# Lalwaniamisha789/Implementation-of-Neural-LDPC-Decoders-with-Degree-Specific-Weight-Sharing-and-RCQ-Quantization

Measured on AMD Instinct MI355X. Metric: decoded codewords/sec at fixed iters; achieved HBM GB/s vs peak, higher is better.
Workload: dtype f32; 1 GPU; (1998,1512) IRA code, BasicMinSumDecoder factor=0.7, fp32, 10 iterations, batch 65536/GPU, SNR 2.0 dB, fixed-iteration flooding decode; graph=ira_1998_1512, n=1998, m=486, edges=6587, batch_per_gpu=65536, global_batch=65536, parallelism=dp1, collective=none

## Files before the change

implementation-of-neural-ldpc-decoders-with-degree-specific-weight-sharing-and-rcq-quantization_amd/_native.py:

```python

from __future__ import annotations

import ctypes as C
import os
import subprocess
import threading
from typing import Optional

import numpy as np

_HERE = os.path.dirname(os.path.abspath(__file__))
LIB_NAME = "libldpc_hip.so"
LIB_PATH = os.environ.get("LDPC_HIP_LIB") or os.path.join(_HERE, LIB_NAME)
CSRC = os.path.join(_HERE, "csrc")
HEADER = os.path.join(os.path.dirname(_HERE), "include", "ldpc_hip.h")
DEBUG_HEADER = os.path.join(os.path.dirname(_HERE), "include", "ldpc_hip_debug.h")

LDPC_F32, LDPC_F64 = 0, 1
C2V_NMS, C2V_RCQ, C2V_OMS = 0, 1, 2
MODE_AUTO, MODE_STREAM, MODE_RESIDENT, MODE_SWEEPS, MODE_GATHER, MODE_PAIR = 0, 1, 2, 3, 4, 5
SCHED_FLOODING, SCHED_LAYERED_REF, SCHED_LAYERED = 0, 1, 2

HIPCC_FLAGS = ["--offload-arch=gfx950", "-O3", "-std=c++17", "-fPIC", "-shared",
               "-ffp-contract=off",
# ... 29 lines not shown
        fn = lib.ldpc_source_hash
        fn.restype = C.c_char_p
        fn.argtypes = []
        return fn().decode() or None
    except (OSError, AttributeError):
        return None


def is_stale(target: Optional[str] = None, defines=()) -> bool:
    target = target or os.path.join(_HERE, LIB_NAME)
    return not os.path.exists(target) or built_hash(target) != source_hash(defines)


def build_native(force: bool = False, verbose: bool = False, defines=(), out: Optional[str] = None) -> str:
    srcs = _source_files()
    target = out or os.path.join(_HERE, LIB_NAME)
    want = source_hash(defines)
    if not force and os.path.exists(target) and built_hash(target) == want:
        return target
    hipcc = os.environ.get("HIPCC") or ("/opt/rocm/bin/hipcc" if os.path.exists("/opt/rocm/bin/hipcc") else "hipcc")
    tmp = target + ".tmp%d" % os.getpid()
    cmd = [hipcc] + HIPCC_FLAGS + [f"-D{d}" for d in defines] + [f"-DLDPC_SRC_HASH={want}", "-o", tmp, srcs[0]]
    res = subprocess.run(cmd, capture_output=True, text=True)
    if verbose or res.returncode != 0:
        print(" ".join(cmd))
        print(res.stdout + res.stderr)
    if res.returncode != 0:
        try:
            os.unlink(tmp)
        except OSError:
            pass
        raise NativeEngineError("hipcc failed:\n" + res.stderr[-4000:])
    os.replace(tmp, target)
    return target


class DecoderDesc(C.Structure):
    _fields_ = [("dtype", C.c_int32), ("c2v_form", C.c_int32), ("iters", C.c_int32),
                ("n_beta_slots", C.c_int32), ("beta", C.c_void_p), ("beta_slot", C.c_void_p),
                ("n_alpha_slots", C.c_int32), ("alpha", C.c_void_p), ("alpha_slot", C.c_void_p),
                ("n_levels", C.c_int32), ("n_quantizers", C.c_int32), ("thresholds", C.c_void_p),
                ("q_of_iter", C.c_void_p),
                ("n_oms_alpha_slots", C.c_int32), ("oms_alpha", C.c_void_p), ("oms_alpha_slot", C.c_void_p),
                ("schedule", C.c_int32)]


PRODUCT_EXPORTS = ("ldpc_graph_create", "ldpc_graph_destroy", "ldpc_graph_info", "ldpc_decoder_create",
                   "ldpc_decoder_set_mode", "ldpc_decoder_info",
                   "ldpc_decoder_set_weights", "ldpc_decoder_destroy", "ldpc_decoder_workspace_bytes",
                   "ldpc_decode", "ldpc_decode_capped", "ldpc_last_error", "ldpc_abi_version", "ldpc_source_hash",
                   "ldpc_train_saved_bytes", "ldpc_train_workspace_bytes", "ldpc_decode_saving", "ldpc_backward",
                   "ldpc_train_joint_workspace_bytes", "ldpc_train_joint")
DEBUG_EXPORTS = ("ldpc_debug_sweep", "ldpc_debug_workspace_layout", "ldpc_debug_resident_c2v", "ldpc_debug_key4",
                 "ldpc_debug_compact_layout", "ldpc_debug_compact_checks")
EXPORTS = PRODUCT_EXPORTS + DEBUG_EXPORTS

_lib = None
_lock = threading.Lock()


def load():
    global _lib
    if _lib is not None:
        return _lib
    with _lock:
        if _lib is not None:
            return _lib
        if not os.path.exists(LIB_PATH):
            raise NativeEngineError(
                f"{LIB_NAME} is not built: run `python -c 'import __graft_entry__ as g; g.build()'` "
                f"(hipcc --offload-arch=gfx950) -- there is no CPU fallback for the decode path")
        if "LDPC_HIP_LIB" not in os.environ and is_stale(LIB_PATH):
            raise NativeEngineError(
                f"{LIB_PATH} was not built from the sources in csrc/ (content hash {built_hash(LIB_PATH)} != "
                f"{source_hash()}): run `python -c 'import __graft_entry__ as g; g.build()'` -- a stale engine is never loaded")
        try:
            lib = C.CDLL(LIB_PATH)
        except OSError as e:
            raise NativeEngineError(f"cannot load {LIB_PATH}: {e}") from e
        vp, i32, i64 = C.c_void_p, C.c_int32, C.c_int64
        lib.ldpc_graph_create.restype = C.c_int
        lib.ldpc_graph_create.argtypes = [C.POINTER(vp), i32, i32, i32, vp, vp]
        lib.ldpc_graph_destroy.restype = None
        lib.ldpc_graph_destroy.argtypes = [vp]
        lib.ldpc_graph_info.restype = C.c_int
        lib.ldpc_graph_info.argtypes = [vp, vp]
        lib.ldpc_decoder_create.restype = C.c_int
        lib.ldpc_decoder_create.argtypes = [C.POINTER(vp), vp, C.POINTER(DecoderDesc)]
        lib.ldpc_decoder_set_mode.restype = C.c_int
        lib.ldpc_decoder_set_mode.argtypes = [vp, i32]
        lib.ldpc_decoder_info.restype = C.c_int
        lib.ldpc_decoder_info.argtypes = [vp, vp]
        lib.ldpc_decoder_set_weights.restype = C.c_int
        lib.ldpc_decoder_set_weights.argtypes = [vp, vp, vp, vp, vp]
        lib.ldpc_decoder_destroy.restype = None
        lib.ldpc_decoder_destroy.argtypes = [vp]
        lib.ldpc_decoder_workspace_bytes.restype = C.c_size_t
        lib.ldpc_decoder_workspace_bytes.argtypes = [vp, i64]
        lib.ldpc_decode.restype = C.c_int
        lib.ldpc_decode.argtypes = [vp, vp, i64, i32, vp, vp, vp, vp, vp, vp, C.c_size_t, vp]
        lib.ldpc_decode_capped.restype = C.c_int
        lib.ldpc_decode_capped.argtypes = [vp, vp, i64, i32, i32, vp, vp, vp, vp, vp, vp, C.c_size_t, vp]
        lib.ldpc_debug_sweep.restype = C.c_int
        lib.ldpc_debug_sweep.argtypes = [vp, i64, i32, i32, vp, C.c_size_t, vp]
        lib.ldpc_debug_workspace_layout.restype = C.c_int
        lib.ldpc_debug_workspace_layout.argtypes = [vp, i64, i32, vp]
        lib.ldpc_debug_key4.restype = C.c_int
        lib.ldpc_debug_key4.argtypes = [vp, i64, C.c_float, vp, vp, vp, vp]
        lib.ldpc_debug_resident_c2v.restype = C.c_int
        lib.ldpc_debug_resident_c2v.argtypes = [vp, vp, i64, i32, i32, vp, vp, vp, vp]
        lib.ldpc_debug_compact_layout.restype = C.c_int
        lib.ldpc_debug_compact_layout.argtypes = [vp, i32, i32, i32, vp, vp, vp, vp, vp]
        lib.ldpc_debug_compact_checks.restype = C.c_int
        lib.ldpc_debug_compact_checks.argtypes = [vp, i32, i32, i32, vp, vp, vp]
        lib.ldpc_train_saved_bytes.restype = C.c_size_t
        lib.ldpc_train_saved_bytes.argtypes = [vp, i64]
        lib.ldpc_train_workspace_bytes.restype = C.c_size_t
        lib.ldpc_train_workspace_bytes.argtypes = [vp, i64]
        lib.ldpc_decode_saving.restype = C.c_int
        lib.ldpc_decode_saving.argtypes = [vp, vp, i64, i32, vp, vp, vp, vp, vp, C.c_size_t, vp, C.c_size_t, vp]
        lib.ldpc_backward.restype = C.c_int
        lib.ldpc_backward.argtypes = [vp, vp, C.c_size_t, vp, i64, vp, vp, vp, vp, vp, vp, vp, C.c_size_t, vp]
        lib.ldpc_train_joint_workspace_bytes.restype = C.c_size_t
        lib.ldpc_train_joint_workspace_bytes.argtypes = [vp, i64]
        lib.ldpc_train_joint.restype = C.c_int
        lib.ldpc_train_joint.argtypes = [vp, vp, vp, i64, vp, vp, vp, vp, vp, vp, vp, vp, vp, C.c_size_t, vp]
        lib.ldpc_last_error.restype = C.c_char_p
        lib.ldpc_last_error.argtypes = []
        lib.ldpc_abi_version.restype = C.c_int
        lib.ldpc_abi_version.argtypes = []
        lib.ldpc_source_hash.restype = C.c_char_p
        lib.ldpc_source_hash.argtypes = []
        if lib.ldpc_abi_version() != 1:
            raise NativeEngineError("libldpc_hip.so ABI version mismatch")
        _lib = lib
    return _lib


def check(rc: int, what: str):
    if rc != 0:
        msg = load().ldpc_last_error().decode(errors="replace")
        if rc == -3:
            raise NotImplementedError(f"{what}: {msg}")
        if rc == -1:
            raise ValueError(f"{what}: {msg}")
        raise NativeEngineError(f"{what} failed (rc={rc}): {msg}")


def ptr(a: Optional[np.ndarray]):
    return None if a is None else a.ctypes.data_as(C.c_void_p)
```

implementation-of-neural-ldpc-decoders-with-degree-specific-weight-sharing-and-rcq-quantization_amd/csrc/ldpc_hip.hip:

```cpp
#include "ldpc_kernels.hip"
#include "ldpc_resident.hip"
#include "ldpc_train.hip"
#include "ldpc_layered.hip"

#include <algorithm>
#include <climits>
#include <mutex>
#include <set>
#include <cmath>
#include <cstdarg>
#include <cstdio>
#include <cstdlib>
#include <cstring>
#include <exception>
#include <new>
#include <vector>

#include "../../include/ldpc_hip.h"
#include "../../include/ldpc_hip_debug.h"

using namespace ldpc;

namespace {

// ... 5 lines not shown
    va_start(ap, fmt);
    vsnprintf(g_err, sizeof(g_err), fmt, ap);
    va_end(ap);
    return code;
}

#define HIP_TRY(expr)                                                                         \
    do {                                                                                      \
        hipError_t e_ = (expr);                                                               \
        if (e_ != hipSuccess) return fail(LDPC_ERR_HIP, "%s -> %s", #expr, hipGetErrorString(e_)); \
    } while (0)

constexpr size_t kAlign = 256;
size_t align_up(size_t x) { return (x + kAlign - 1) / kAlign * kAlign; }

template <typename X>
int upload(X **dst, const X *src, size_t count)
{
    *dst = nullptr;
    if (count == 0) count = 1;
    HIP_TRY(hipMalloc((void **)dst, count * sizeof(X)));
    if (src) HIP_TRY(hipMemcpy(*dst, src, count * sizeof(X), hipMemcpyHostToDevice));
    return LDPC_OK;
}

struct DeviceGuard {
    int prev = -1;
    bool switched = false;
    explicit DeviceGuard(int dev)
    {
        if (hipGetDevice(&prev) == hipSuccess && prev != dev) switched = hipSetDevice(dev) == hipSuccess;
    }
    ~DeviceGuard()
    {
        if (switched) (void)hipSetDevice(prev);
    }
};

}

struct ldpc_graph {
    int device = 0;
    int n = 0, m = 0, E = 0, max_dc = 0, max_dv = 0;
    int *check_ptr = nullptr, *var_idx = nullptr, *var_ptr = nullptr, *csc_edge = nullptr;
    int *wide_checks = nullptr;
    int n_wide = 0;
    std::vector<int> h_check_ptr, h_var_idx, h_var_ptr, h_csc, h_check_of_edge;
    GraphDev dev() const { return GraphDev{n, m, E, check_ptr, var_idx, var_ptr, csc_edge}; }
};

constexpr int kCptWaves = kResCptThreads / 64;
constexpr int kCptCells = kCptWaves * kResRegVars;
constexpr int kCptMaxDv = 8;
inline int cpt_body_cost(int dv) { return dv * (dv - 1) + 2 * dv + 4; }

struct CptLayout {
    std::vector<int> var_at;
    unsigned cell[kCptWaves] = {};
    int worst = 0, total = 0;
    int mixed = 0;
};

struct ldpc_decoder {
    const ldpc_graph *g = nullptr;
    int dtype = LDPC_F32, form = LDPC_C2V_NMS, T = 0;
    int n_beta = 0, n_alpha = 0, n_levels = 0, n_quant = 0, n_oms_alpha = 0;
    void *beta = nullptr, *alpha = nullptr, *oms_alpha = nullptr;
    int *beta_slot = nullptr, *alpha_slot = nullptr, *oms_alpha_slot = nullptr;
    float *thresholds = nullptr;
    float *lut = nullptr;
    std::vector<int> q_of_iter;
    int *q_of_iter_dev = nullptr;
    size_t elem() const { return dtype == LDPC_F64 ? 8 : 4; }
    int schedule = 0;
    int mode = 0;
    bool res_ok = false;
    int res_G = 0, res_NT = 0;
    bool unit_alpha = false, rcq_zero0 = false;
    bool beta_per_check = false;
    size_t res_lds = 0;
    ResidentPlan res{};
    bool resc_ok = false;
    size_t resc_lds = 0;
    ResidentPlan resc{};
    CptLayout resc_layout;
    std::vector<void *> res_bufs;
    int *beta_inv_ptr = nullptr, *beta_inv_items = nullptr;
    int *alpha_inv_ptr = nullptr, *alpha_inv_items = nullptr;
    int *oms_inv_ptr = nullptr, *oms_inv_items = nullptr;
    bool gat_ok = false;
    bool pair_ok = false;
    bool key_float4 = false;
    int4 *gat_meta = nullptr;
    int *gat_nbr = nullptr;
    bool lay_ok = false;
    LayeredPlan lay{};
    uint32_t *lay_off = nullptr;
    size_t lay_lds = 0;
    int *lay_slot = nullptr;
    float *lay_beta = nullptr;
    bool beta_unit = false;
};

namespace {

bool use_resident(const ldpc_decoder *d) { return d->res_ok && (d->mode == LDPC_MODE_AUTO || d->mode == LDPC_MODE_RESIDENT); }
bool use_layered_lds(const ldpc_decoder *d) { return d->lay_ok && (d->mode == LDPC_MODE_AUTO || d->mode == LDPC_MODE_RESIDENT); }
bool use_pair(const ldpc_decoder *d) { return d->pair_ok && d->mode != LDPC_MODE_SWEEPS && d->mode != LDPC_MODE_GATHER; }
bool use_gather(const ldpc_decoder *d) { return d->gat_ok && !use_pair(d) && d->mode != LDPC_MODE_SWEEPS && d->mode != LDPC_MODE_PAIR; }

int pick_vec(const ldpc_decoder *d, int64_t batch)
{
    if (batch <= 64) return 1;
// ... 821 lines not shown
    for (bool improved = true; improved;) {
        improved = false;
        for (int x = 0; x < kCptCells; ++x)
            for (int y = x + 1; y < kCptCells; ++y) {
                const int wx = x / kResRegVars, rx = x % kResRegVars, wy = y / kResRegVars, ry = y % kResRegVars;
                const int cx = slot[wx][rx], cy = slot[wy][ry];
                if (wx == wy || (cx < 0 && cy < 0)) continue;
                if ((cx >= 0 && hi(cells[cx]) && ry != 0) || (cy >= 0 && hi(cells[cy]) && rx != 0)) continue;
                long long m0, s0, m1, s1;
                objective(m0, s0);
                const int kx = cx >= 0 ? cost(cells[cx]) : 0, ky = cy >= 0 ? cost(cells[cy]) : 0;
                load[wx] += ky - kx; load[wy] += kx - ky;
                objective(m1, s1);
                if (m1 < m0 || (m1 == m0 && s1 < s0)) { std::swap(slot[wx][rx], slot[wy][ry]); improved = true; }
                else { load[wx] -= ky - kx; load[wy] -= kx - ky; }
            }
    }
    int by_load[kCptWaves];
    for (int w = 0; w < kCptWaves; ++w) by_load[w] = w;
    std::stable_sort(by_load, by_load + kCptWaves, [&](int x, int y) { return load[x] > load[y]; });
    int wave_of[kCptWaves];
    for (int k = 0; k < kCptWaves / 2; ++k) {
        wave_of[k] = by_load[k];
        wave_of[k + kCptWaves / 2] = by_load[kCptWaves - 1 - k];
    }
    std::vector<std::vector<int>> of_deg(kCptMaxDv + 1);
    for (int j = 0; j < n; ++j) of_deg[dv[j]].push_back(j);
    size_t taken[kCptMaxDv + 1] = {};
    L.var_at.assign((size_t)kCptCells * 64, -1);
    for (int w = 0; w < kCptWaves; ++w) {
        int cs[kResRegVars];
        for (int r = 0; r < kResRegVars; ++r) cs[r] = slot[wave_of[w]][r];
        std::stable_sort(cs, cs + kResRegVars, [&](int x, int y) {
            if (x < 0 || y < 0) return x >= 0 && y < 0;
            if (hi(cells[x]) != hi(cells[y])) return hi(cells[x]);
            return cost(cells[x]) > cost(cells[y]);
        });
        for (int r = 0; r < kResRegVars; ++r) {
            if (cs[r] < 0) continue;
            int lane = 0;
            for (int d = kCptMaxDv; d >= 0; --d)
                for (int k = 0; k < cells[cs[r]].cnt[d]; ++k)
                    L.var_at[(size_t)r * kResCptThreads + w * 64 + lane++] = of_deg[d][taken[d]++];
        }
    }
    int n_pos = 0;
    for (int q = 0; q < (int)L.var_at.size(); ++q)
        if (L.var_at[q] >= 0) n_pos = q + 1;
    L.var_at.resize((size_t)n_pos);
    cpt_cells(dv, L);
    return true;
}

void cpt_lane_order(std::vector<int> &var_at, const std::vector<std::vector<int>> &vs, int G)
{
    const int n = (int)vs.size() - 1;
    std::vector<int> order(var_at.size());
    for (size_t q = 0; q < var_at.size(); ++q) order[q] = var_at[q] >= 0 ? var_at[q] : n;
    LaneCost lc{vs, order, 32, 32, G == 2 ? 16 : 32, G == 2 ? 16 : 32};
    std::vector<std::vector<int>> classes(kCptMaxDv + 1);
    for (int q = 0; q < (int)order.size(); ++q) {
        const int d = (int)vs[order[q]].size();
        if (order[q] != n && d > 0 && d <= kCptMaxDv) classes[d].push_back(q);
    }
    classes.erase(std::remove_if(classes.begin(), classes.end(), [](const std::vector<int> &c) { return c.size() < 2; }),
                  classes.end());
    if (classes.empty()) return;
    uint64_t rng = 0x9E3779B97F4A7C15ull;
    auto next = [&]() { rng ^= rng << 13; rng ^= rng >> 7; rng ^= rng << 17; return rng; };
    const long trials = std::min<long>(400000, 150L * n);
    for (long it = 0; it < trials; ++it) {
        const auto &c = classes[next() % classes.size()];
        const int x = c[next() % c.size()], y = c[next() % c.size()];
        if (x / lc.wg == y / lc.wg) continue;
        const int before = lc.around(x, y);
        std::swap(order[x], order[y]);
        if (lc.around(x, y) > before) std::swap(order[x], order[y]);
    }
    for (size_t q = 0; q < var_at.size(); ++q) var_at[q] = order[q] == n ? -1 : order[q];
}

struct ResVCheck { int check, e0, dc, gs; };
int resident_layout(ldpc_decoder *d, const ldpc_decoder_desc *desc, const std::vector<ResVCheck> &vc, int mstride,
                    long long S, int G, ResidentPlan &pl, const CptLayout *cl = nullptr);
void cpt_layout(const ldpc_graph *g, const std::vector<ResVCheck> &vc, long long S, CptLayout &L);
void cpt_check_words(const std::vector<ResVCheck> &vc, bool select_form, unsigned (&words)[kCptWaves]);
bool cpt_geometry(const ldpc_graph *g, const std::vector<ResVCheck> &vc, long long &Sc);

bool resident_checks(const ldpc_graph *g, std::vector<ResVCheck> &vc)
{
    auto dc_real = [&](int i) { return g->h_check_ptr[i + 1] - g->h_check_ptr[i]; };
    std::vector<int> wide_ids, plain_ids;
    for (int i = 0; i < g->m; ++i) (dc_real(i) > kResSubDegreeCap ? wide_ids : plain_ids).push_back(i);
    auto group_of = [&](int i) { int k = 1; while (k * kResSubDegree < dc_real(i)) k <<= 1; return k; };
    for (int i : wide_ids)
        if (group_of(i) > 64) return false;
    std::stable_sort(wide_ids.begin(), wide_ids.end(), [&](int a, int b) { return group_of(a) > group_of(b); });
    for (int i : wide_ids) {
        const int k = group_of(i), dc = dc_real(i), base = dc / k, rem = dc % k;
        int e = g->h_check_ptr[i];
        for (int j = 0; j < k; ++j) {
            const int len = base + (j < rem ? 1 : 0);
            vc.push_back({i, e, len, k});
            e += len;
        }
    }
    std::stable_sort(plain_ids.begin(), plain_ids.end(), [&](int a, int b) { return dc_real(a) > dc_real(b); });
    for (int i : plain_ids) vc.push_back({i, g->h_check_ptr[i], dc_real(i), 1});
    return true;
}

int build_resident_plan(ldpc_decoder *d, const ldpc_decoder_desc *desc)
{
    const ldpc_graph *g = d->g;
    d->res_ok = false;
    if (g->E == 0 || g->max_dv > 8) return LDPC_OK;
    const bool f64 = d->dtype == LDPC_F64;
    if (f64 && (d->form != LDPC_C2V_NMS || !d->beta_per_check)) return LDPC_OK;
    const int n = g->n;
    if (n > 65535 || d->n_beta > 65535 || d->n_alpha >= (1 << 24) || d->n_oms_alpha > 65535) return LDPC_OK;

    std::vector<ResVCheck> vc;
    if (!resident_checks(g, vc)) return LDPC_OK;
    const int m = (int)vc.size();
    int max_sub = 0;
    for (const ResVCheck &v : vc) max_sub = std::max(max_sub, v.dc);
    if (m > 65535 || max_sub > 255) return LDPC_OK;

    auto geometry = [&](int stride, int &G_out, int &blocks_out) {
        const long long S_ = (long long)max_sub * stride;
        const int mp = is_pow2(stride) ? m : 0;
        if (S_ > 65535 || !resident_fits(d, S_, 1, 1, mp)) return false;
        const int G_ = resident_fits(d, S_, 2, 1, mp) ? 2 : 1;
        int b_ = 1;
        while (b_ < 8 && resident_fits(d, S_, G_, b_ + 1, mp)) ++b_;
// ... 4 lines not shown
    if (!geometry(m, G, blocks)) return LDPC_OK;
    if (f64 && G != 2) return LDPC_OK;
    if (m <= 512) {
        int G5 = 0, b5 = 0;
        if (geometry(512, G5, b5) && G5 == G && std::min(b5, 2) == std::min(blocks, 2)) { mstride = 512; blocks = b5; }
    }
    const long long S = (long long)max_sub * mstride;
    const int NT = blocks >= 2 ? 512 : 1024;
    if (int rc = resident_layout(d, desc, vc, mstride, S, G, d->res)) return rc;
    d->res_G = G; d->res_NT = NT;
    d->res_lds = res_lds_total((int)S, n, G, resident_alpha_floats(d), d->res.par_words);
    d->res_ok = true;

    d->resc_ok = false;
    long long Sc = 0;
    if (!f64 && G == 2 && NT == kResCptThreads && cpt_geometry(g, vc, Sc)) {
        cpt_layout(g, vc, Sc, d->resc_layout);
        if (int rc = resident_layout(d, desc, vc, kResCptStride, Sc, 2, d->resc, &d->resc_layout)) return rc;
        d->resc_lds = res_cpt_lds_total((int)Sc, 2);
        d->resc_ok = true;
    }
    return LDPC_OK;
}

bool cpt_geometry(const ldpc_graph *g, const std::vector<ResVCheck> &vc, long long &Sc)
{
    const int n = g->n, m = (int)vc.size();
    int max_sub = 0;
    for (const ResVCheck &v : vc) max_sub = std::max(max_sub, v.dc);
    if (m != g->m || m > kResCptStride || n > kResRegVars * kResCptThreads || g->max_dv > kCptMaxDv || max_sub < 1)
        return false;
    int n_top = 0;
    while (n_top < m && vc[n_top].dc == max_sub) ++n_top;
    Sc = (long long)(max_sub - 1) * kResCptStride + n_top;
    int n_hi = 0;
    for (int j = 0; j < n; ++j) n_hi += (g->h_var_ptr[j + 1] - g->h_var_ptr[j]) > 4 ? 1 : 0;
    return Sc * 2 * 4 <= 65535 && (long long)n <= Sc && n_hi <= kResCptThreads &&
           kResCptBlocks * res_cpt_lds_total((int)Sc, 2) <= kLdsBytes;
}

void cpt_check_words(const std::vector<ResVCheck> &vc, bool select_form, unsigned (&words)[kCptWaves])
{
    const int m = (int)vc.size();
    for (int w = 0; w < kCptWaves; ++w) {
        const int p0 = std::min(64 * w, m), p1 = std::min(p0 + 64, m);
        int lo = p0 < p1 ? 255 : 0, hi = 0;
        for (int p = p0; p < p1; ++p) { lo = std::min(lo, vc[p].dc); hi = std::max(hi, vc[p].dc); }
        words[w] = p0 < p1 ? chk_word(lo, hi, p1 - p0) | (select_form ? 0u : kChkPerLane) : 0u;
    }
}

void cpt_layout(const ldpc_graph *g, const std::vector<ResVCheck> &vc, long long S, CptLayout &L)
{
    const int n = g->n, m = (int)vc.size();
    std::vector<int> dv(n);
    for (int j = 0; j < n; ++j) dv[j] = g->h_var_ptr[j + 1] - g->h_var_ptr[j];
    std::vector<int> slot_of_edge(g->E);
    for (int p = 0; p < m; ++p)
        for (int t = 0; t < vc[p].dc; ++t) slot_of_edge[vc[p].e0 + t] = t * kResCptStride + p;
    std::vector<std::vector<int>> vs(n + 1);
    for (int j = 0; j < n; ++j)
        for (int k = 0; k < dv[j]; ++k) vs[j].push_back(slot_of_edge[g->h_csc[g->h_var_ptr[j] + k]]);
    if (!cpt_assign(dv, L) || (long long)L.var_at.size() > S) {
        L.var_at.resize(n);
        for (int j = 0; j < n; ++j) L.var_at[j] = j;
        std::stable_sort(L.var_at.begin(), L.var_at.end(), [&](int a, int b) { return dv[a] > dv[b]; });
    }
    cpt_lane_order(L.var_at, vs, 2);
    cpt_cells(dv, L);
}

int resident_layout(ldpc_decoder *d, const ldpc_decoder_desc *desc, const std::vector<ResVCheck> &vc, int mstride,
                    long long S, int G, ResidentPlan &pl, const CptLayout *cl)
{
    const ldpc_graph *g = d->g;
    const int n = g->n, m = (int)vc.size();
    const bool any_split = m != g->m;
    int max_sub = 0;
    for (const ResVCheck &v : vc) max_sub = std::max(max_sub, v.dc);
    std::vector<int> perm_v(n), pos_v(n);
    for (int j = 0; j < n; ++j) perm_v[j] = j;
    auto dv_of = [&](int j) { return g->h_var_ptr[j + 1] - g->h_var_ptr[j]; };
    std::stable_sort(perm_v.begin(), perm_v.end(), [&](int a, int b) { return dv_of(a) > dv_of(b); });
    std::vector<int> slot_of_edge(g->E);
    for (int p = 0; p < m; ++p)
        for (int t = 0; t < vc[p].dc; ++t) slot_of_edge[vc[p].e0 + t] = t * mstride + p;
    if (cl) {
        perm_v = cl->var_at;
    } else {
        std::vector<std::vector<int>> vs(n);
        for (int j = 0; j < n; ++j)
            for (int k = 0; k < dv_of(j); ++k) vs[j].push_back(slot_of_edge[g->h_csc[g->h_var_ptr[j] + k]]);
        optimise_lane_order(perm_v, vs, G);
    }
    const int n_pos = (int)perm_v.size();
    const int n_ent = cl ? (n_pos + 63) / 64 * 64 : n;
    for (int q = 0; q < n_pos; ++q)
        if (perm_v[q] >= 0) pos_v[perm_v[q]] = q;

    std::vector<uint8_t> dc_s(m), gsz(m);
    std::vector<uint16_t> cvar((size_t)S, 0), bslot((size_t)S, 0), oaslot((size_t)S, 0), bslot_c(m, 0), inv(n);
    std::vector<uint32_t> vmeta(n_ent, 0u);
    std::vector<uint2> vslot_lo(n_ent, make_uint2(0, kResHole)), vslot_hi(std::max(n_ent, 1), make_uint2(0, 0));
    int n_hi = 0;
    std::vector<uint32_t> edge_of_slot((size_t)S, 0xffffffffu);
    bool per_check = true;
    for (int p = 0; p < m; ++p) {
        const ResVCheck &v = vc[p];
        const int first = g->h_check_ptr[v.check];
        dc_s[p] = (uint8_t)v.dc;
        gsz[p] = (uint8_t)v.gs;
        for (int t = 0; t < v.dc; ++t) {
            const int e = v.e0 + t, slot = t * mstride + p;
            edge_of_slot[slot] = (uint32_t)e;
            cvar[slot] = (uint16_t)pos_v[g->h_var_idx[e]];
            bslot[slot] = (uint16_t)desc->beta_slot[e];
            if (desc->beta_slot[e] != desc->beta_slot[first]) per_check = false;
            if (d->form == LDPC_C2V_OMS && desc->oms_alpha) oaslot[slot] = (uint16_t)desc->oms_alpha_slot[e];
        }
        bslot_c[p] = v.dc ? (uint16_t)desc->beta_slot[first] : 0;
    }
    for (int q = 0; q < n_pos; ++q) {
        if (perm_v[q] < 0) continue;
        const int j = perm_v[q], s0 = g->h_var_ptr[j], dv = dv_of(j);
        vmeta[q] = (uint32_t)dv | ((uint32_t)desc->alpha_slot[j] << 8);
        inv[j] = (uint16_t)q;
        uint32_t off[8] = {0, 0, 0, 0, 0, 0, 0, 0};
        for (int k = 0; k < dv; ++k) off[k] = (uint32_t)slot_of_edge[g->h_csc[s0 + k]] * G * 4;
        vslot_lo[q] = make_uint2(off[0] | (off[1] << 16), off[2] | (off[3] << 16));
        vslot_hi[q] = make_uint2(off[4] | (off[5] << 16), off[6] | (off[7] << 16));
        if (dv > 4) n_hi = q + 1;
    }
    pl = ResidentPlan{};
    pl.n = n; pl.m = m; pl.S = (int)S; pl.max_dc = max_sub; pl.max_dv = g->max_dv; pl.mstride = mstride; pl.E = g->E;
    pl.any_split = any_split ? 1 : 0;
    pl.n_hi = n_hi;
    pl.n_pos = n_pos;
    if (cl) {
        std::copy(cl->cell, cl->cell + kCptWaves, pl.vcell);
        cpt_check_words(vc, per_check && (d->form == LDPC_C2V_NMS || (d->form == LDPC_C2V_RCQ && d->rcq_zero0)),
                        pl.ccell);
    }
    pl.par_words = is_pow2(mstride) ? m : 0;
    pl.par_shift = G == 2 ? 3 : 2;
    int rc = plan_upload(d, &pl.dc_s, dc_s);
    if (!rc && any_split) rc = plan_upload(d, &pl.gsz, gsz);
    if (!rc) rc = plan_upload(d, &pl.cvar, cvar);
    if (!rc) rc = plan_upload(d, &pl.bslot, bslot);
    if (!rc && per_check) rc = plan_upload(d, &pl.bslot_c, bslot_c);
    if (!rc && d->form == LDPC_C2V_OMS && desc->oms_alpha) rc = plan_upload(d, &pl.oaslot, oaslot);
    if (!rc) rc = plan_upload(d, &pl.vmeta, vmeta);
    if (!rc) rc = plan_upload(d, &pl.vslot_lo, vslot_lo);
    vslot_hi.resize((size_t)std::max(n_hi, 1));
    if (!rc) rc = plan_upload(d, &pl.vslot_hi, vslot_hi);
    if (!rc) rc = plan_upload(d, &pl.inv_perm_v, inv);
    if (!rc) rc = plan_upload(d, &pl.edge_of_slot, edge_of_slot);
    return rc;
}

int allow_full_lds(const void *kfn, int device)
{
    static std::mutex mu;
    static std::set<std::pair<const void *, int>> done;
    std::lock_guard<std::mutex> lk(mu);
    if (done.count({kfn, device})) return LDPC_OK;
    HIP_TRY(hipFuncSetAttribute(kfn, hipFuncAttributeMaxDynamicSharedMemorySize, (int)kLdsBytes));
// ... 1017 lines not shown
        if (int rc = graph_host_build(&g, n, m, E, check_ptr, var_idx)) return rc;
        std::vector<ResVCheck> vc;
        long long Sc = 0;
        if (!resident_checks(&g, vc) || !cpt_geometry(&g, vc, Sc))
            return fail(LDPC_ERR_UNSUPPORTED, "the graph does not qualify for the compact plan");
        cpt_layout(&g, vc, Sc, own);
    }
    if (pos_of_var) {
        for (int j = 0; j < n; ++j) pos_of_var[j] = -1;
        for (int q = 0; q < (int)L->var_at.size(); ++q)
            if (L->var_at[q] >= 0) pos_of_var[L->var_at[q]] = q;
    }
    if (cells)
        for (int c = 0; c < kCptCells; ++c) cells[c] = (uint8_t)(L->cell[c / kResRegVars] >> (8 * (c % kResRegVars)));
    if (stats) {
        stats[0] = (int32_t)L->var_at.size(); stats[1] = L->worst; stats[2] = L->total; stats[3] = L->mixed;
    }
    return LDPC_OK;
}

int ldpc_debug_compact_layout(const ldpc_decoder *d, int32_t n, int32_t m, int32_t E, const int32_t *check_ptr,
                              const int32_t *var_idx, int32_t *pos_of_var, uint8_t cells[32], int32_t stats[4])
{
    LDPC_NOTHROW(compact_layout_impl(d, n, m, E, check_ptr, var_idx, pos_of_var, cells, stats))
}

static int compact_checks_impl(const ldpc_decoder *d, int32_t n, int32_t m, int32_t E, const int32_t *check_ptr,
                               const int32_t *var_idx, uint32_t *words)
{
    if (!words) return fail(LDPC_ERR_ARG, "NULL argument");
    if (d) {
        if (!d->resc_ok) return fail(LDPC_ERR_UNSUPPORTED, "the decoder has no compact fixed-T plan");
        std::copy(d->resc.ccell, d->resc.ccell + kCptWaves, words);
        return LDPC_OK;
    }
    ldpc_graph g;
    if (int rc = graph_host_build(&g, n, m, E, check_ptr, var_idx)) return rc;
    std::vector<ResVCheck> vc;
    long long Sc = 0;
    if (!resident_checks(&g, vc) || !cpt_geometry(&g, vc, Sc))
        return fail(LDPC_ERR_UNSUPPORTED, "the graph does not qualify for the compact plan");
    unsigned own[kCptWaves];
    cpt_check_words(vc, true, own);
    std::copy(own, own + kCptWaves, words);
    return LDPC_OK;
}

int ldpc_debug_compact_checks(const ldpc_decoder *d, int32_t n, int32_t m, int32_t E, const int32_t *check_ptr,
                              const int32_t *var_idx, uint32_t words[8])
{
    LDPC_NOTHROW(compact_checks_impl(d, n, m, E, check_ptr, var_idx, words))
}

int ldpc_debug_resident_c2v(const ldpc_decoder *d, const void *llr, int64_t batch, int32_t early_stop,
                            int32_t max_iterations, void *posterior, int32_t *iterations, void *c2v_out, void *stream)
{
    if (!d || !llr || !posterior || !c2v_out || batch <= 0) return fail(LDPC_ERR_ARG, "bad argument");
    if (!use_resident(d)) return fail(LDPC_ERR_ARG, "the decoder is not on the LDS-resident engine");
    if (d->g->n == 0) return LDPC_OK;
    IterCap cap(max_iterations > 0 ? max_iterations : INT_MAX);
    return decode_resident(d, llr, batch, early_stop, nullptr, posterior, iterations, nullptr, nullptr, c2v_out, stream);
}

int ldpc_debug_sweep(const ldpc_decoder *d, int64_t batch, int32_t which, int32_t iter, void *workspace,
                     size_t workspace_bytes, void *stream)
{
    if (!d || !workspace || batch <= 0) return fail(LDPC_ERR_ARG, "bad argument");
    if (iter < 0 || iter >= d->T) return fail(LDPC_ERR_ARG, "iter outside [0, T)");
    if (use_resident(d) || use_layered_lds(d)) return fail(LDPC_ERR_ARG, "debug sweeps need LDPC_MODE_STREAM");
    const Workspace w = carve(d, batch, workspace);
    if (w.total > workspace_bytes) return fail(LDPC_ERR_WORKSPACE, "workspace too small");
    DeviceGuard guard(d->g->device);
    hipStream_t s = (hipStream_t)stream;
    const bool f64 = d->dtype == LDPC_F64;
    if (use_pair(d) && !f64) {
        if (which == 0 && (iter >= 1 || (w.vec == 4 && pair_q4<4>(d))))
            return w.vec == 1 ? launch_cn_q<1>(d, w, iter, false, s) : launch_cn_q<4>(d, w, iter, false, s);
        if (which != 0 && iter < d->T - 1) return w.vec == 1 ? launch_vn_q<1>(d, w, iter, false, s) : launch_vn_q<4>(d, w, iter, false, s);
    }
    if (use_gather(d) && !f64) {
        char *buf[2] = {w.c2v, w.v2c};
        if (which == 0 && iter >= 1)
            return w.vec == 1 ? launch_gather<1>(d, w, iter, false, buf[(iter - 1) & 1], buf[iter & 1], s)
                              : launch_gather<4>(d, w, iter, false, buf[(iter - 1) & 1], buf[iter & 1], s);
        if (which != 0) {
            Workspace wv = w;
            wv.c2v = buf[iter & 1];
            return w.vec == 1 ? launch_vn<float, 1>(d, wv, iter, true, false, s) : launch_vn<float, 4>(d, wv, iter, true, false, s);
        }
    }
#define LDPC_DBG(REAL_, V_)                                                                 \
    return which == 0 ? launch_cn<REAL_, V_>(d, w, iter, false, s)                           \
                      : launch_vn<REAL_, V_>(d, w, iter, iter == d->T - 1, false, s)
    if (f64) {
        if (w.vec == 1) { LDPC_DBG(double, 1); } else { LDPC_DBG(double, 2); }
    } else {
        if (w.vec == 1) { LDPC_DBG(float, 1); } else { LDPC_DBG(float, 4); }
    }
#undef LDPC_DBG
}

}
```

implementation-of-neural-ldpc-decoders-with-degree-specific-weight-sharing-and-rcq-quantization_amd/csrc/ldpc_resident.hip:

```cpp
#pragma once

#include "ldpc_kernels.hip"

namespace ldpc {

struct ResidentPlan {
    int n, m, S, max_dc, max_dv;
    int mstride;
    const uint8_t *dc_s;
    const uint8_t *gsz;
    int any_split;
    int par_words;
    int par_shift;
    const uint16_t *cvar;
    const uint16_t *bslot;
    const uint16_t *bslot_c;
    const uint16_t *oaslot;
    const uint32_t *vmeta;
    const uint2 *vslot_lo;
    const uint2 *vslot_hi;
    int n_hi;
    const uint16_t *inv_perm_v;
    int n_pos;
    unsigned vcell[8];
// ... 882 lines not shown
                const bool in = j < n;
                const unsigned bb = bits_s[ip[k]];
#pragma unroll
                for (int g = 0; g < G; ++g) {
                    if (!((mask >> g) & 1u)) continue;
                    const unsigned bit = (bb >> g) & 1u;
                    if (in && a.bits) res_stream_store(&a.bits[(size_t)(b0 + g) * n + j], (int)bit);
                    if (a.packed) res_store_packed<G>(a, b0 + g, j, n, in && bit != 0);
                }
            }
        }
    }
    if (tid == 0) {
#pragma unroll
        for (int g = 0; g < G; ++g) {
            if (!((mask >> g) & 1u)) continue;
            if (a.iterations) a.iterations[b0 + g] = iters;
            if (a.success) a.success[b0 + g] = (uint8_t)(((unsat >> g) & 1u) ? 0 : 1);
        }
    }
}

template <int G, typename T>
__device__ __forceinline__ void res_dump_c2v(const ResidentPlan &pl, const ResidentArgs &a, long long b0, unsigned mask,
                                             int tid, int nt)
{
    using P = Pack<T, G>;
    T *out = reinterpret_cast<T *>(a.dbg_c2v);
    for (int s = tid; s < pl.S; s += nt) {
        const unsigned e = pl.edge_of_slot[s];
        if (e == 0xffffffffu) continue;
        const P v = lds_load<P>((unsigned)s * (unsigned)sizeof(P));
#pragma unroll
        for (int g = 0; g < G; ++g)
            if ((mask >> g) & 1u) out[(size_t)(b0 + g) * pl.E + e] = v.x[g];
    }
}

__host__ __device__ inline size_t res_off_llr(int S, int G) { return (size_t)S * G * 4; }
__host__ __device__ inline size_t res_off_alpha(int S, int n, int G) { return res_off_llr(S, G) + (size_t)n * G * 4; }
__host__ __device__ inline size_t res_off_bits(int S, int n, int G, int n_alpha_lds) { return res_off_alpha(S, n, G) + (size_t)n_alpha_lds * 4; }
__host__ __device__ inline size_t res_off_flag(int S, int n, int G, int n_alpha_lds) { return (res_off_bits(S, n, G, n_alpha_lds) + n + 3) / 4 * 4; }
__host__ __device__ inline size_t res_off_par(int S, int n, int G, int n_alpha_lds) { return res_off_flag(S, n, G, n_alpha_lds) + 16; }
__host__ __device__ inline size_t res_lds_total(int S, int n, int G, int n_alpha_lds, int m_par) { return res_off_par(S, n, G, n_alpha_lds) + 4 * (size_t)m_par; }

__host__ __device__ inline size_t res_cpt_off_flag(int S, int G) { return ((size_t)S * G * 4 + 15) / 16 * 16; }
__host__ __device__ inline size_t res_cpt_lds_total(int S, int G) { return res_cpt_off_flag(S, G) + 16; }

constexpr int kResMaxThreads = 1024;
constexpr int kResMinWaves = 4;
constexpr int kResCptThreads = 512;
constexpr int kResCptWaves = 6;
constexpr int kResCptBlocks = 3;
constexpr int kResCptStride = 496;
template <int G, int FORM, bool BPC, int NL, int MS, int ES, typename T = float, bool SPLIT = false, bool REG = false,
          bool CPT = false>
__global__ __launch_bounds__(CPT ? kResCptThreads : kResMaxThreads, CPT ? kResCptWaves : kResMinWaves)
void resident_decode(ResidentPlan pl, ResidentArgs a)
{
    static_assert(!CPT || (REG && !ES && !SPLIT && std::is_same<T, float>::value), "compact: fixed-T fp32 REG kernels only");
    extern __shared__ __align__(16) unsigned char res_smem[];
    if (__builtin_amdgcn_groupstaticsize() != 0) __builtin_trap();
    constexpr int GE = G * (int)(sizeof(T) / 4);
    const int n_alpha_lds = a.alpha_in_lds ? a.T * a.n_alpha * (int)(sizeof(T) / 4) : 0;
    T *llr_s = reinterpret_cast<T *>(res_smem + (CPT ? 0 : res_off_llr(pl.S, GE)));
    T *alpha_s = reinterpret_cast<T *>(res_smem + res_off_alpha(pl.S, pl.n, GE));
    uint8_t *bits_s = res_smem + res_off_bits(pl.S, pl.n, GE, n_alpha_lds);
    unsigned *sh_unsat = reinterpret_cast<unsigned *>(res_smem + (CPT ? res_cpt_off_flag(pl.S, GE)
                                                                        : res_off_flag(pl.S, pl.n, GE, n_alpha_lds)));
    ParScatter ps, psf;
    if (pl.par_words) {
        psf.par_off = (unsigned)res_off_par(pl.S, pl.n, GE, n_alpha_lds);
        psf.shift = (unsigned)pl.par_shift;
        psf.mask = (unsigned)pl.mstride - 1u;
        if (ES) ps = psf;
    }
    const T *g_llr = reinterpret_cast<const T *>(a.llr);
    const T *g_beta = reinterpret_cast<const T *>(a.beta);
    const T *g_alpha = reinterpret_cast<const T *>(a.alpha);
    const T *g_oms_alpha = reinterpret_cast<const T *>(a.oms_alpha);
    using P = Pack<T, G>;
    const int tid = threadIdx.x, nt = blockDim.x, n = pl.n;
    const long long b0 = (long long)blockIdx.x * G;
    constexpr unsigned kAll = (1u << G) - 1u;

    constexpr int kPro = 4;
    for (int j0 = tid; j0 < n; j0 += kPro * nt) {
        unsigned ip[kPro];
        P v[kPro];
#pragma unroll
        for (int k = 0; k < kPro; ++k) {
            const int j = j0 + k * nt;
            ip[k] = 0;
            if (j < n) {
                ip[k] = pl.inv_perm_v[j];
#pragma unroll
                for (int g = 0; g < G; ++g)
                    v[k].x[g] = (b0 + g < a.batch) ? res_stream_load(&g_llr[(size_t)(b0 + g) * n + j]) : (T)1;
            }
        }
#pragma unroll
        for (int k = 0; k < kPro; ++k)
            if (j0 + k * nt < n) reinterpret_cast<P *>(llr_s)[ip[k]] = v[k];
    }
    for (int k = tid; k < (a.alpha_in_lds ? a.T * a.n_alpha : 0); k += nt) alpha_s[k] = g_alpha[k];
    if (tid == 0) { sh_unsat[0] = 0; sh_unsat[1] = 0; }
    for (int k = tid; k < pl.par_words; k += nt) lds_store<unsigned>(psf.par_off + 4u * (unsigned)k, 0u);
// ... 212 lines not shown
```

include/ldpc_hip_debug.h:

```cpp
#ifndef LDPC_HIP_DEBUG_H
#define LDPC_HIP_DEBUG_H

#include "ldpc_hip.h"

#ifdef __cplusplus
extern "C" {
#endif

int ldpc_debug_sweep(const ldpc_decoder *d, int64_t batch, int32_t which, int32_t iter,
                     void *workspace, size_t workspace_bytes, void *stream);

int ldpc_debug_workspace_layout(const ldpc_decoder *d, int64_t batch, int32_t max_iterations, int64_t out8[8]);

int ldpc_debug_resident_c2v(const ldpc_decoder *d, const void *llr, int64_t batch, int32_t early_stop,
                            int32_t max_iterations, void *posterior, int32_t *iterations, void *c2v_out,
                            void *stream);

int ldpc_debug_compact_layout(const ldpc_decoder *d, int32_t n, int32_t m, int32_t E, const int32_t *check_ptr,
                              const int32_t *var_idx, int32_t *pos_of_var, uint8_t cells[32], int32_t stats[4]);

int ldpc_debug_compact_checks(const ldpc_decoder *d, int32_t n, int32_t m, int32_t E, const int32_t *check_ptr,
                              const int32_t *var_idx, uint32_t words[8]);

int ldpc_debug_key4(const float *values, int64_t count, float beta, const float thresholds4[4], uint8_t *keys_float,
                    uint8_t *keys_compare, void *stream);

#ifdef __cplusplus
}
#endif
#endif
```

Before: 33.80 million codewords/s.

## Jointly optimize variable, check and row slot placement for LDS bank conflicts

Replaces the variable-only lane-order search in the compact resident plan with an incremental LDS bank-conflict cost model. A local search now also swaps same-degree check positions and reorders edge rows within a check, and it accepts ties that lower a sum-of-squares term. The resulting check order and per-edge slots feed the kernel layout. The check stride changes from 496 to 495, which is likely meant to break power-of-two bank aliasing. Host-side planning time grows with up to several million trials, and a debug export is added to inspect the bank model.

```diff
diff --git a/implementation-of-neural-ldpc-decoders-with-degree-specific-weight-sharing-and-rcq-quantization_amd/_native.py b/implementation-of-neural-ldpc-decoders-with-degree-specific-weight-sharing-and-rcq-quantization_amd/_native.py
--- a/implementation-of-neural-ldpc-decoders-with-degree-specific-weight-sharing-and-rcq-quantization_amd/_native.py
+++ b/implementation-of-neural-ldpc-decoders-with-degree-specific-weight-sharing-and-rcq-quantization_amd/_native.py
@@ -105,7 +105,7 @@
                    "ldpc_train_saved_bytes", "ldpc_train_workspace_bytes", "ldpc_decode_saving", "ldpc_backward",
                    "ldpc_train_joint_workspace_bytes", "ldpc_train_joint")
 DEBUG_EXPORTS = ("ldpc_debug_sweep", "ldpc_debug_workspace_layout", "ldpc_debug_resident_c2v", "ldpc_debug_key4",
-                 "ldpc_debug_compact_layout", "ldpc_debug_compact_checks")
+                 "ldpc_debug_compact_layout", "ldpc_debug_compact_checks", "ldpc_debug_compact_banks")
 EXPORTS = PRODUCT_EXPORTS + DEBUG_EXPORTS
 
 _lib = None
@@ -164,6 +164,8 @@
         lib.ldpc_debug_resident_c2v.argtypes = [vp, vp, i64, i32, i32, vp, vp, vp, vp]
         lib.ldpc_debug_compact_layout.restype = C.c_int
         lib.ldpc_debug_compact_layout.argtypes = [vp, i32, i32, i32, vp, vp, vp, vp, vp]
+        lib.ldpc_debug_compact_banks.restype = C.c_int
+        lib.ldpc_debug_compact_banks.argtypes = [vp, i32, i32, i32, vp, vp, vp, vp, vp, vp, vp, vp, vp]
         lib.ldpc_debug_compact_checks.restype = C.c_int
         lib.ldpc_debug_compact_checks.argtypes = [vp, i32, i32, i32, vp, vp, vp]
         lib.ldpc_train_saved_bytes.restype = C.c_size_t
diff --git a/implementation-of-neural-ldpc-decoders-with-degree-specific-weight-sharing-and-rcq-quantization_amd/csrc/ldpc_hip.hip b/implementation-of-neural-ldpc-decoders-with-degree-specific-weight-sharing-and-rcq-quantization_amd/csrc/ldpc_hip.hip
--- a/implementation-of-neural-ldpc-decoders-with-degree-specific-weight-sharing-and-rcq-quantization_amd/csrc/ldpc_hip.hip
+++ b/implementation-of-neural-ldpc-decoders-with-degree-specific-weight-sharing-and-rcq-quantization_amd/csrc/ldpc_hip.hip
@@ -81,6 +81,7 @@
 constexpr int kCptWaves = kResCptThreads / 64;
 constexpr int kCptCells = kCptWaves * kResRegVars;
 constexpr int kCptMaxDv = 8;
+constexpr long kCptJointTrials = 3000000;
 inline int cpt_body_cost(int dv) { return dv * (dv - 1) + 2 * dv + 4; }
 
 struct CptLayout {
@@ -88,6 +89,8 @@
     unsigned cell[kCptWaves] = {};
     int worst = 0, total = 0;
     int mixed = 0;
+    std::vector<int> check_at, slot_of_edge, base_check_at, base_slot_of_edge;
+    int banks[4] = {}, base_banks[4] = {};
 };
 
 struct ldpc_decoder {
@@ -1015,35 +1018,186 @@
     return true;
 }
 
-void cpt_lane_order(std::vector<int> &var_at, const std::vector<std::vector<int>> &vs, int G)
-{
-    const int n = (int)vs.size() - 1;
-    std::vector<int> order(var_at.size());
-    for (size_t q = 0; q < var_at.size(); ++q) order[q] = var_at[q] >= 0 ? var_at[q] : n;
-    LaneCost lc{vs, order, 32, 32, G == 2 ? 16 : 32, G == 2 ? 16 : 32};
-    std::vector<std::vector<int>> classes(kCptMaxDv + 1);
-    for (int q = 0; q < (int)order.size(); ++q) {
-        const int d = (int)vs[order[q]].size();
-        if (order[q] != n && d > 0 && d <= kCptMaxDv) classes[d].push_back(q);
-    }
-    classes.erase(std::remove_if(classes.begin(), classes.end(), [](const std::vector<int> &c) { return c.size() < 2; }),
-                  classes.end());
-    if (classes.empty()) return;
+struct ResVCheck { int check, e0, dc, gs; };
+
+struct BankModel {
+    static constexpr int kRG = 32, kRM = 32, kWG = 16, kWM = 16;
+    const ldpc_graph *g;
+    const std::vector<ResVCheck> &vc;
+    std::vector<int> &var_at, &check_at, &slot_of_edge;
+    std::vector<int> pos_of_var, k_of_edge, edge_at;
+    std::vector<unsigned char> hist[2], mx[2];
+    std::vector<int> dirty;
+    long long cost = 0, sq = 0;
+
+    BankModel(const ldpc_graph *g_, const std::vector<ResVCheck> &vc_, std::vector<int> &var_at_,
+              std::vector<int> &check_at_, std::vector<int> &slot_of_edge_)
+        : g(g_), vc(vc_), var_at(var_at_), check_at(check_at_), slot_of_edge(slot_of_edge_)
+    {
+        const int n_pos = (int)var_at.size();
+        pos_of_var.assign(g->n, -1);
+        for (int q = 0; q < n_pos; ++q)
+            if (var_at[q] >= 0) pos_of_var[var_at[q]] = q;
+        k_of_edge.assign(g->E, 0);
+        for (int j = 0; j < g->n; ++j)
+            for (int s = g->h_var_ptr[j]; s < g->h_var_ptr[j + 1]; ++s) k_of_edge[g->h_csc[s]] = s - g->h_var_ptr[j];
+        edge_at.assign(g->E, 0);
+        for (const ResVCheck &v : vc)
+            for (int t = 0; t < v.dc; ++t) edge_at[v.e0 + t] = v.e0 + t;
+        const int rcells = (n_pos + kRG - 1) / kRG * kCptMaxDv, wcells = (n_pos + kWG - 1) / kWG * kCptMaxDv;
+        hist[0].assign((size_t)rcells * kRM, 0); mx[0].assign(rcells, 0);
+        hist[1].assign((size_t)wcells * kWM, 0); mx[1].assign(wcells, 0);
+        for (int e = 0; e < g->E; ++e) entry(e, +1);
+        settle();
+    }
+    void bump(int kind, int cell, int banks, int bank, int sign)
+    {
+        unsigned char &c = hist[kind][(size_t)cell * banks + bank];
+        if (sign > 0) {
+            sq += 2 * c + 1;
+            if (++c > mx[kind][cell]) { mx[kind][cell] = c; ++cost; }
+        } else {
+            sq -= 2 * c - 1;
+            if (c-- == mx[kind][cell]) dirty.push_back(kind | cell << 1);
+        }
+    }
+    void entry(int e, int sign)
+    {
+        const int q = pos_of_var[g->h_var_idx[e]], k = k_of_edge[e], s = slot_of_edge[e];
+        bump(0, q / kRG * kCptMaxDv + k, kRM, s % kRM, sign);
+        bump(1, q / kWG * kCptMaxDv + k, kWM, s % kWM, sign);
+    }
+    void settle()
+    {
+        for (int dc : dirty) {
+            const int kind = dc & 1, cell = dc >> 1, banks = kind ? kWM : kRM;
+            const unsigned char *h = &hist[kind][(size_t)cell * banks];
+            unsigned char m = 0;
+            for (int b = 0; b < banks; ++b) m = std::max(m, h[b]);
+            cost += (int)m - (int)mx[kind][cell];
+            mx[kind][cell] = m;
+        }
+        dirty.clear();
+    }
+    void swap_vars(int x, int y)
+    {
+        const int jx = var_at[x], jy = var_at[y];
+        for (int j : {jx, jy})
+            for (int s = g->h_var_ptr[j]; s < g->h_var_ptr[j + 1]; ++s) entry(g->h_csc[s], -1);
+        std::swap(var_at[x], var_at[y]);
+        pos_of_var[jx] = y; pos_of_var[jy] = x;
+        for (int j : {jx, jy})
+            for (int s = g->h_var_ptr[j]; s < g->h_var_ptr[j + 1]; ++s) entry(g->h_csc[s], +1);
+        settle();
+    }
+    void swap_checks(int p, int r)
+    {
+        const ResVCheck &a = vc[check_at[p]], &b = vc[check_at[r]];
+        for (int t = 0; t < a.dc; ++t) { entry(a.e0 + t, -1); entry(b.e0 + t, -1); }
+        for (int t = 0; t < a.dc; ++t) { slot_of_edge[a.e0 + t] += r - p; slot_of_edge[b.e0 + t] += p - r; }
+        for (int t = 0; t < a.dc; ++t) { entry(a.e0 + t, +1); entry(b.e0 + t, +1); }
+        std::swap(check_at[p], check_at[r]);
+        settle();
+    }
+    void swap_rows(int p, int t, int u)
+    {
+        const ResVCheck &a = vc[check_at[p]];
+        const int e = edge_at[a.e0 + t], f = edge_at[a.e0 + u];
+        entry(e, -1); entry(f, -1);
+        std::swap(slot_of_edge[e], slot_of_edge[f]);
+        std::swap(edge_at[a.e0 + t], edge_at[a.e0 + u]);
+        entry(e, +1); entry(f, +1);
+        settle();
+    }
+    void report(int (&out)[4]) const
+    {
+        for (int kind = 0; kind < 2; ++kind) {
+            int c = 0, groups = 0;
+            for (unsigned char m : mx[kind]) { c += m; groups += m ? 1 : 0; }
+            out[2 * kind] = c; out[2 * kind + 1] = groups;
+        }
+    }
+};
+
+void cpt_place_banks(const ldpc_graph *g, const std::vector<ResVCheck> &vc, CptLayout &L)
+{
+    const int n = g->n, m = (int)vc.size();
+    L.check_at.resize(m);
+    L.slot_of_edge.assign(g->E, 0);
+    for (int p = 0; p < m; ++p) {
+        L.check_at[p] = p;
+        for (int t = 0; t < vc[p].dc; ++t) L.slot_of_edge[vc[p].e0 + t] = t * kResCptStride + p;
+    }
+    BankModel bm(g, vc, L.var_at, L.check_at, L.slot_of_edge);
+    std::vector<std::vector<int>> vclass(kCptMaxDv + 1);
+    for (int q = 0; q < (int)L.var_at.size(); ++q) {
+        if (L.var_at[q] < 0) continue;
+        const int d = g->h_var_ptr[L.var_at[q] + 1] - g->h_var_ptr[L.var_at[q]];
+        if (d > 0 && d <= kCptMaxDv) vclass[d].push_back(q);
+    }
+    vclass.erase(std::remove_if(vclass.begin(), vclass.end(), [](const std::vector<int> &c) { return c.size() < 2; }),
+                 vclass.end());
+    std::vector<std::pair<int, int>> cclass;
+    std::vector<int> rowable;
+    for (int p = 0; p < m;) {
+        int r = p;
+        while (r < m && vc[r].dc == vc[p].dc) ++r;
+        if (r - p >= 2 && vc[p].dc > 0) cclass.push_back({p, r});
+        p = r;
+    }
+    for (int p = 0; p < m; ++p)
+        if (vc[p].dc >= 2) rowable.push_back(p);
     uint64_t rng = 0x9E3779B97F4A7C15ull;
     auto next = [&]() { rng ^= rng << 13; rng ^= rng >> 7; rng ^= rng << 17; return rng; };
-    const long trials = std::min<long>(400000, 150L * n);
-    for (long it = 0; it < trials; ++it) {
-        const auto &c = classes[next() % classes.size()];
-        const int x = c[next() % c.size()], y = c[next() % c.size()];
-        if (x / lc.wg == y / lc.wg) continue;
-        const int before = lc.around(x, y);
-        std::swap(order[x], order[y]);
-        if (lc.around(x, y) > before) std::swap(order[x], order[y]);
-    }
-    for (size_t q = 0; q < var_at.size(); ++q) var_at[q] = order[q] == n ? -1 : order[q];
-}
-
-struct ResVCheck { int check, e0, dc, gs; };
+    if (!vclass.empty()) {
+        const long trials = std::min<long>(400000, 150L * n);
+        for (long it = 0; it < trials; ++it) {
+            const auto &c = vclass[next() % vclass.size()];
+            const int x = c[next() % c.size()], y = c[next() % c.size()];
+            if (x / BankModel::kWG == y / BankModel::kWG) continue;
+            const long long before = bm.cost;
+            bm.swap_vars(x, y);
+            if (bm.cost > before) bm.swap_vars(x, y);
+        }
+    }
+    bm.report(L.base_banks);
+    L.base_check_at = L.check_at;
+    L.base_slot_of_edge = L.slot_of_edge;
+
+    const long joint = std::min<long>(kCptJointTrials, 500L * g->E);
+    for (long it = 0; it < joint; ++it) {
+        const long long cost0 = bm.cost, sq0 = bm.sq;
+        const unsigned kind = (unsigned)(next() % 32);
+        int a = 0, b = 0, c = 0;
+        if (kind < 2) {
+            if (vclass.empty()) continue;
+            const auto &cl = vclass[next() % vclass.size()];
+            a = cl[next() % cl.size()]; b = cl[next() % cl.size()];
+            if (a / BankModel::kWG == b / BankModel::kWG) continue;
+            bm.swap_vars(a, b);
+        } else if (kind < 3) {
+            if (cclass.empty()) continue;
+            const auto &cl = cclass[next() % cclass.size()];
+            a = cl.first + (int)(next() % (uint64_t)(cl.second - cl.first));
+            b = cl.first + (int)(next() % (uint64_t)(cl.second - cl.first));
+            if (a == b) continue;
+            bm.swap_checks(a, b);
+        } else {
+            if (rowable.empty()) continue;
+            a = rowable[next() % rowable.size()];
+            const int dc = vc[L.check_at[a]].dc;
+            b = (int)(next() % (uint64_t)dc); c = (int)(next() % (uint64_t)dc);
+            if (b == c) continue;
+            bm.swap_rows(a, b, c);
+        }
+        if (bm.cost < cost0 || (bm.cost == cost0 && bm.sq <= sq0)) continue;
+        if (kind < 2) bm.swap_vars(a, b);
+        else if (kind < 3) bm.swap_checks(a, b);
+        else bm.swap_rows(a, b, c);
+    }
+    bm.report(L.banks);
+}
+
 int resident_layout(ldpc_decoder *d, const ldpc_decoder_desc *desc, const std::vector<ResVCheck> &vc, int mstride,
                     long long S, int G, ResidentPlan &pl, const CptLayout *cl = nullptr);
 void cpt_layout(const ldpc_graph *g, const std::vector<ResVCheck> &vc, long long S, CptLayout &L);
@@ -1154,28 +1308,26 @@
 
 void cpt_layout(const ldpc_graph *g, const std::vector<ResVCheck> &vc, long long S, CptLayout &L)
 {
-    const int n = g->n, m = (int)vc.size();
+    const int n = g->n;
     std::vector<int> dv(n);
     for (int j = 0; j < n; ++j) dv[j] = g->h_var_ptr[j + 1] - g->h_var_ptr[j];
-    std::vector<int> slot_of_edge(g->E);
-    for (int p = 0; p < m; ++p)
-        for (int t = 0; t < vc[p].dc; ++t) slot_of_edge[vc[p].e0 + t] = t * kResCptStride + p;
-    std::vector<std::vector<int>> vs(n + 1);
-    for (int j = 0; j < n; ++j)
-        for (int k = 0; k < dv[j]; ++k) vs[j].push_back(slot_of_edge[g->h_csc[g->h_var_ptr[j] + k]]);
     if (!cpt_assign(dv, L) || (long long)L.var_at.size() > S) {
         L.var_at.resize(n);
         for (int j = 0; j < n; ++j) L.var_at[j] = j;
         std::stable_sort(L.var_at.begin(), L.var_at.end(), [&](int a, int b) { return dv[a] > dv[b]; });
     }
-    cpt_lane_order(L.var_at, vs, 2);
+    cpt_place_banks(g, vc, L);
     cpt_cells(dv, L);
 }
 
-int resident_layout(ldpc_decoder *d, const ldpc_decoder_desc *desc, const std::vector<ResVCheck> &vc, int mstride,
+int resident_layout(ldpc_decoder *d, const ldpc_decoder_desc *desc, const std::vector<ResVCheck> &sorted, int mstride,
                     long long S, int G, ResidentPlan &pl, const CptLayout *cl)
 {
     const ldpc_graph *g = d->g;
+    std::vector<ResVCheck> placed;
+    if (cl)
+        for (int c : cl->check_at) placed.push_back(sorted[c]);
+    const std::vector<ResVCheck> &vc = cl ? placed : sorted;
     const int n = g->n, m = (int)vc.size();
     const bool any_split = m != g->m;
     int max_sub = 0;
@@ -1189,6 +1341,7 @@
         for (int t = 0; t < vc[p].dc; ++t) slot_of_edge[vc[p].e0 + t] = t * mstride + p;
     if (cl) {
         perm_v = cl->var_at;
+        slot_of_edge = cl->slot_of_edge;
     } else {
         std::vector<std::vector<int>> vs(n);
         for (int j = 0; j < n; ++j)
@@ -1213,7 +1366,7 @@
         dc_s[p] = (uint8_t)v.dc;
         gsz[p] = (uint8_t)v.gs;
         for (int t = 0; t < v.dc; ++t) {
-            const int e = v.e0 + t, slot = t * mstride + p;
+            const int e = v.e0 + t, slot = slot_of_edge[e];
             edge_of_slot[slot] = (uint32_t)e;
             cvar[slot] = (uint16_t)pos_v[g->h_var_idx[e]];
             bslot[slot] = (uint16_t)desc->beta_slot[e];
@@ -2337,6 +2490,51 @@
     LDPC_NOTHROW(compact_checks_impl(d, n, m, E, check_ptr, var_idx, words))
 }
 
+static int compact_banks_impl(const ldpc_decoder *d, int32_t n, int32_t m, int32_t E, const int32_t *check_ptr,
+                              const int32_t *var_idx, int32_t *slot_of_edge, int32_t *pos_of_check, int32_t *model,
+                              int32_t *base_slot_of_edge, int32_t *base_pos_of_check, int32_t *base_model,
+                              int32_t *geometry)
+{
+    CptLayout own;
+    ldpc_graph own_g;
+    const CptLayout *L = &own;
+    const ldpc_graph *g = &own_g;
+    std::vector<ResVCheck> vc;
+    long long Sc = 0;
+    if (d) {
+        if (!d->resc_ok) return fail(LDPC_ERR_UNSUPPORTED, "the decoder has no compact fixed-T plan");
+        L = &d->resc_layout;
+        g = d->g;
+        Sc = d->resc.S;
+        if (!resident_checks(g, vc)) return fail(LDPC_ERR_UNSUPPORTED, "the graph does not qualify for the compact plan");
+    } else {
+        if (int rc = graph_host_build(&own_g, n, m, E, check_ptr, var_idx)) return rc;
+        if (!resident_checks(g, vc) || !cpt_geometry(g, vc, Sc))
+            return fail(LDPC_ERR_UNSUPPORTED, "the graph does not qualify for the compact plan");
+        cpt_layout(g, vc, Sc, own);
+    }
+    auto emit = [&](const std::vector<int> &slots, const std::vector<int> &check_at, const int (&banks)[4],
+                    int32_t *slots_out, int32_t *pos_out, int32_t *model_out) {
+        if (slots_out) std::copy(slots.begin(), slots.end(), slots_out);
+        if (pos_out)
+            for (int p = 0; p < (int)check_at.size(); ++p) pos_out[vc[check_at[p]].check] = p;
+        if (model_out) std::copy(banks, banks + 4, model_out);
+    };
+    emit(L->slot_of_edge, L->check_at, L->banks, slot_of_edge, pos_of_check, model);
+    emit(L->base_slot_of_edge, L->base_check_at, L->base_banks, base_slot_of_edge, base_pos_of_check, base_model);
+    if (geometry) { geometry[0] = kResCptStride; geometry[1] = (int32_t)Sc; }
+    return LDPC_OK;
+}
+
+int ldpc_debug_compact_banks(const ldpc_decoder *d, int32_t n, int32_t m, int32_t E, const int32_t *check_ptr,
+                             const int32_t *var_idx, int32_t *slot_of_edge, int32_t *pos_of_check, int32_t model[4],
+                             int32_t *base_slot_of_edge, int32_t *base_pos_of_check, int32_t base_model[4],
+                             int32_t geometry[2])
+{
+    LDPC_NOTHROW(compact_banks_impl(d, n, m, E, check_ptr, var_idx, slot_of_edge, pos_of_check, model, base_slot_of_edge,
+                                    base_pos_of_check, base_model, geometry))
+}
+
 int ldpc_debug_resident_c2v(const ldpc_decoder *d, const void *llr, int64_t batch, int32_t early_stop,
                             int32_t max_iterations, void *posterior, int32_t *iterations, void *c2v_out, void *stream)
 {
diff --git a/implementation-of-neural-ldpc-decoders-with-degree-specific-weight-sharing-and-rcq-quantization_amd/csrc/ldpc_resident.hip b/implementation-of-neural-ldpc-decoders-with-degree-specific-weight-sharing-and-rcq-quantization_amd/csrc/ldpc_resident.hip
--- a/implementation-of-neural-ldpc-decoders-with-degree-specific-weight-sharing-and-rcq-quantization_amd/csrc/ldpc_resident.hip
+++ b/implementation-of-neural-ldpc-decoders-with-degree-specific-weight-sharing-and-rcq-quantization_amd/csrc/ldpc_resident.hip
@@ -958,7 +958,7 @@
 constexpr int kResCptThreads = 512;
 constexpr int kResCptWaves = 6;
 constexpr int kResCptBlocks = 3;
-constexpr int kResCptStride = 496;
+constexpr int kResCptStride = 495;
 template <int G, int FORM, bool BPC, int NL, int MS, int ES, typename T = float, bool SPLIT = false, bool REG = false,
           bool CPT = false>
 __global__ __launch_bounds__(CPT ? kResCptThreads : kResMaxThreads, CPT ? kResCptWaves : kResMinWaves)
diff --git a/include/ldpc_hip_debug.h b/include/ldpc_hip_debug.h
--- a/include/ldpc_hip_debug.h
+++ b/include/ldpc_hip_debug.h
@@ -22,6 +22,11 @@
 int ldpc_debug_compact_checks(const ldpc_decoder *d, int32_t n, int32_t m, int32_t E, const int32_t *check_ptr,
                               const int32_t *var_idx, uint32_t words[8]);
 
+int ldpc_debug_compact_banks(const ldpc_decoder *d, int32_t n, int32_t m, int32_t E, const int32_t *check_ptr,
+                             const int32_t *var_idx, int32_t *slot_of_edge, int32_t *pos_of_check, int32_t model[4],
+                             int32_t *base_slot_of_edge, int32_t *base_pos_of_check, int32_t base_model[4],
+                             int32_t geometry[2]);
+
 int ldpc_debug_key4(const float *values, int64_t count, float beta, const float thresholds4[4], uint8_t *keys_float,
                     uint8_t *keys_compare, void *stream);
 
```

Measured after the change: 35.21 million codewords/s (median of 6 runs). 1.04x the previous value.
